# josl/kmerjs

Measured on AMD Instinct MI355X. Metric: k-mers/sec + distinct-kmers/sec, k=16 150bp synthetic FASTQ, 1/2/4/8 GPU, higher is better.
Workload: dtype u8; 1 GPU; C2: 10000000 synthetic 150bp reads per GPU, k=16, prefix 'ATGAC'; reads_per_gpu=10000000, mode=ordered (reference Map insertion order), k=16, prefix=ATGAC, bytes_per_gpu=3170000000, pipeline=off (steps in sequence), parallelism=dp1 (one GPU; no collective), backend=none

## Files before the change

### kmerjs_amd/csrc/kmer_api.hip

```cpp
#include "kmer_host.hpp"

using namespace kmerhip;

extern "C" {

const char *kmer_version(void) { return "kmerhip 0.2 (gfx950)"; }

const char *kmer_status_string(kmer_status s) {
    switch (s) {
    case KMER_OK: return "ok";
    case KMER_E_IO: return "i/o error";
    case KMER_E_BAD_PARAM: return "bad parameter";
    case KMER_E_OOM: return "out of memory";
    case KMER_E_DEVICE: return "device error";
    case KMER_E_TOO_MANY_KEYS: return "too many keys";
    case KMER_E_NONASCII: return "non-ASCII input";
    case KMER_E_LINE_TOO_LONG: return "line too long";
    case KMER_E_STATE: return "bad call sequence";
    }
    return "unknown";
}

const char *kmer_last_error(const kmer_ctx *ctx) { return ctx ? ctx->err.c_str() : "null context"; }

// ... 297 lines not shown
kmer_status kmer_feed_device(kmer_ctx *c, const void *d_bytes, size_t len, void *stream) {
    if (!c || (!d_bytes && len)) return KMER_E_BAD_PARAM;
    SETTLE(c);
    if (!c->open_stream) return fail(c, KMER_E_STATE, "feed without reset");
    if (hipSetDevice(c->device) != hipSuccess) return KMER_E_DEVICE;
    hipStream_t s = (hipStream_t)stream;
    if (s != c->stream) {
        HIPCHK(c, hipEventRecord(c->evw, s));
        HIPCHK(c, hipStreamWaitEvent(c->stream, c->evw, 0));
    }
    return feed(c, (const uint8_t *)d_bytes, len, c->stream);
}

kmer_status kmer_finish_device(kmer_ctx *c, kmer_result **out) {
    if (!c) return KMER_E_BAD_PARAM;
    SETTLE(c);
    if (hipSetDevice(c->device) != hipSuccess) return KMER_E_DEVICE;
    if (out) *out = nullptr;
    return finish(c, out);
}


kmer_status kmer_partial_device(kmer_ctx *c, const void **d_keys, const void **d_vals, uint64_t *n) {
    if (!c || !d_keys || !d_vals || !n) return KMER_E_BAD_PARAM;
    SETTLE(c);
    if (c->mode != MODE_PACKED && c->mode != MODE_WINDOWS)
        return fail(c, KMER_E_STATE, "configuration has no packed keys");
    if (c->wide) return fail(c, KMER_E_STATE, "keys of 64 bits or more (k - |P| >= 32) have no packed partials");
    if (hipSetDevice(c->device) != hipSuccess) return KMER_E_DEVICE;
    kmer_status st = apply_cross(c);
    if (st) return st;
// ... 1572 lines not shown
```

### kmerjs_amd/csrc/kmer_feed.hip

```cpp
#include "kmer_host.hpp"

namespace kmerhip {

kmer_status ensure_tiles(kmer_ctx *c, uint64_t n_tiles) {
    if (n_tiles <= c->tile_cap) return KMER_OK;
    const uint64_t cap = std::max<uint64_t>(n_tiles, 1024);
    hipStream_t s = c->stream;
    if (c->mode == MODE_TABLE) {
    } else if (c->mode == MODE_GENERAL || c->mode == MODE_WINDOWS) {
        HIPCHK(c, c->lb_cnt.ensure(cap, s));
        HIPCHK(c, c->lb_lnl.ensure(cap, s));
        HIPCHK(c, c->tp_cnt.ensure(cap, s));
        HIPCHK(c, c->tp_lnl.ensure(cap, s));
    } else {
        HIPCHK(c, c->tsum.ensure(cap, s));
        HIPCHK(c, c->tscan.ensure(cap, s));
        HIPCHK(c, c->bsum.ensure(cap / TSCAN_BLOCK + 2, s));
        HIPCHK(c, c->bscan.ensure(cap / TSCAN_BLOCK + 2, s));
        HIPCHK(c, c->hits.ensure(cap * HMAX, s));
        if (c->p.k > 32) HIPCHK(c, c->hits_hi.ensure(cap * HMAX, s));
    }
    c->tile_cap = cap;
    return KMER_OK;
}
// ... 47 lines not shown
    HIPCHK(c, hipStreamSynchronize(s));
    std::string key;
    for (uint64_t i = 0; i < n; ++i) {
        key.assign(keys.data() + i * k, recs[i].len);
        auto it = c->exotic.find(key);
        if (it == c->exotic.end()) {
            c->exotic.emplace(key, Ent{1, recs[i].order});
        } else {
            it->second.count += 1;
            it->second.first = std::min(it->second.first, recs[i].order);
        }
    }
    return KMER_OK;
}

kmer_status wait_tail(kmer_ctx *c, uint64_t seq, hipStream_t qs) {
    volatile uint64_t *flag = c->h_tail + 9;
    for (uint32_t i = 1;; ++i) {
        if (__atomic_load_n(flag, __ATOMIC_ACQUIRE) == seq) break;
        if ((i & 1023) == 0) {
            const hipError_t e = hipStreamQuery(qs);
            if (e == hipSuccess) {
                if (__atomic_load_n(flag, __ATOMIC_ACQUIRE) == seq) break;
                return fail(c, KMER_E_DEVICE, "chunk counters were not published");
            }
            if (e != hipErrorNotReady) HIPCHK(c, e);
        }
        __builtin_ia32_pause();
    }
    memcpy(c->h_small, (const void *)c->h_tail, 8 * 8);
    return KMER_OK;
}

static void take_chunk_stamps(kmer_ctx *c) {
    const uint64_t t0 = c->h_tail[TAIL_STAMP + STAMP_SCAN_START], t1 = c->h_tail[TAIL_STAMP + STAMP_SCAN_END],
                   t2 = c->h_tail[TAIL_STAMP + STAMP_FEED_END];
    c->scan_ms += (double)(int64_t)(t1 - t0) / c->clock_khz;
    c->feed_ms += (double)(int64_t)(t2 - t0) / c->clock_khz;
}

kmer_status flush_prep(kmer_ctx *c, hipStream_t s, uint32_t extra) {
    const uint32_t f = c->prep_flags | extra;
    if (!f) return KMER_OK;
    HIPCHK(c, launch_prep(c->d_pos, c->d_pos_saved, c->d_err, c->d_scal, f, c->prep_lines, c->d_stamp, s));
    c->prep_flags = 0;
// ... 50 lines not shown
    h.xbase = c->n_cross;
    h.xcap = c->xord.cap;
    uint64_t rcap = c->narrow ? c->rkey32.cap : c->rkey.cap;
    rcap = std::min<uint64_t>(rcap, c->rord.cap);
    if (c->wide) rcap = std::min<uint64_t>(rcap, c->rkeyh.cap);
    h.rcap = rcap;
}

kmer_status launch_chunk(kmer_ctx *c) {
    auto &p = c->pend;
    const hipStream_t s = p.s;
    uint64_t *stamp = c->d_stamp;
    if (c->planes) HIPCHK(c, launch_scan_planes(p.a, c->pargs, s));
    else HIPCHK(c, launch_scan_tiles(p.a, s));
    HIPCHK(c, launch_tile_reduce(c->tsum.p, p.n_tiles, c->bsum.p, stamp, s));
    if (p.n_blocks > TSCAN_INLINE_MAX) {
        TileSum zero;
        memset(&zero, 0, sizeof(zero));
        ROCPRIM_RUN(c, rocprim::exclusive_scan(t, b, c->bsum.p, c->bscan.p, zero, (size_t)p.n_blocks, TileSumOp(), s));
        HIPCHK(c, launch_tile_scan(c->tsum.p, p.n_tiles, c->bscan.p, true, p.init, c->tscan.p, s));
    } else {
        HIPCHK(c, launch_tile_scan(c->tsum.p, p.n_tiles, c->bsum.p, false, p.init, c->tscan.p, s));
    }
    p.h.seq = ++c->tail_seq;
    p.h.stamp = stamp;
    HIPCHK(c, launch_hits(p.h, s));
    if (c->mode == MODE_PACKED && !c->wide)
        HIPCHK(c, launch_cross_segsort_chunk(p.h.xord, p.h.xkey, p.h.xslot, p.h.xbase, p.h.xcap, c->d_xcount,
                                             c->d_cross_go, p.h.rkey, p.h.rkey32, p.h.rord, c->pbits, s));
    if (s != c->stream) {
        HIPCHK(c, hipEventRecord(c->evw, s));
        HIPCHK(c, hipStreamWaitEvent(c->stream, c->evw, 0));
    }
    return KMER_OK;
}

kmer_status scan_feed(kmer_ctx *c, const uint8_t *d, uint64_t len, uint32_t n_tiles, hipStream_t s) {
    const bool packed = c->mode == MODE_PACKED;
    kmer_status st;
// ... 729 lines not shown
```

### kmerjs_amd/csrc/kmer_finish.hip

```cpp
#include "kmer_host.hpp"

namespace kmerhip {

kmer_status apply_cross(kmer_ctx *c) {
    hipStream_t s = c->stream;
    const uint64_t n = c->n_cross;
    if (n == 0) return KMER_OK;
    uint32_t *k32 = c->narrow ? c->rkey32.p : nullptr;
    if (!c->long_seg) {
        HIPCHK(c, launch_cross_segsort(c->xord.p, c->xkey.p, c->xslot.p, n, c->rkey.p, k32, c->rord.p, c->pbits,
                                       c->fin_stamp, s));
        c->fin_stamp = nullptr;
    } else if (n <= XSMALL_MAX) {
        HIPCHK(c, launch_cross_sort_small(c->xslot.p, c->xord.p, c->xkey.p, n, c->rkey.p, k32, c->rord.p, s));
    } else {
        StreamPos pos;
        kmer_status st = read_pos(c, &pos);
        if (st) return st;
        HIPCHK(c, c->xord2.ensure(n, s));
        HIPCHK(c, c->xkey2.ensure(n, s));
        rocprim::double_buffer<uint64_t> ob(c->xord.p, c->xord2.p);
        rocprim::double_buffer<uint64_t> kb(c->xkey.p, c->xkey2.p);
        const int obits = std::min(64, bit_width(((pos.lines + 1) << (c->pbits + 1)) | ((2ull << c->pbits) - 1ull)));
        ROCPRIM_RUN(c, rocprim::radix_sort_pairs(t, b, ob, kb, (size_t)n, 0, obits, s));
// ... 38 lines not shown
    rocprim::counting_iterator<uint32_t> iota(0u);
    ROCPRIM_RUN(c, rocprim::radix_sort_pairs(t, b, c->rkey.p, c->rkey2.p, iota, c->ridx2.p, (size_t)n, 0, 64, s));
    HIPCHK(c, launch_gather_u64(c->rkeyh.p, c->ridx2.p, n, c->whA.p, s));
    const int hbits = (int)c->kbits - 64 + 1;
    ROCPRIM_RUN(c, rocprim::radix_sort_pairs(t, b, c->whA.p, c->whB.p, c->ridx2.p, c->ridx3.p, (size_t)n, 0, hbits, s));
    HIPCHK(c, launch_gather_u64(c->rkey.p, c->ridx3.p, n, c->rkey2.p, s));
    HIPCHK(c, hipMemsetD32Async((hipDeviceptr_t)c->hcnt.p, 1, n, s));
    HIPCHK(c, launch_heads_wide(c->whB.p, c->rkey2.p, c->ridx3.p, n, 1ull << (c->kbits - 64), c->hcnt.p, s));
    return KMER_OK;
}

bool bucket_route(const kmer_ctx *c, bool with_counts) {
    return c->narrow && c->kbits <= BKT_LOW + 11 && !with_counts && !(c->p.flags & KMER_FLAG_SORT_FINISH);
}

kmer_status bucket_heads(kmer_ctx *c, uint64_t n, bool partial) {
    hipStream_t s = c->stream;
    const uint32_t shift = std::min<uint32_t>(c->kbits, BKT_LOW);
    const uint32_t nb = 1u << (c->kbits - shift);
    const uint64_t nblk64 = (n + BKT_EPB_HOST - 1) / BKT_EPB_HOST;
    if (nblk64 > 0x7FFFFFFFull) return fail(c, KMER_E_BAD_PARAM, "too many hits");
    const uint32_t nblk = (uint32_t)nblk64;
    const uint32_t invalid = 1u << c->kbits;
    uint64_t *stamp = c->fin_stamp;
    c->fin_stamp = nullptr;
    const uint64_t cap = bucket_cap(n, nb);
    if (!c->bkt_counted && (uint64_t)nb * cap <= 0x7FFFFFFFull) {
        HIPCHK(c, c->pkey16.ensure((uint64_t)nb * cap, s));
        HIPCHK(c, c->ridx2.ensure((uint64_t)nb * cap, s));
        if (!c->bcur.p) {
            HIPCHK(c, c->bcur.ensure((uint64_t)BKT_MAX * BKT_CUR_STRIDE, s));
            HIPCHK(c, hipMemsetAsync(c->bcur.p, 0, (uint64_t)BKT_MAX * BKT_CUR_STRIDE * sizeof(uint32_t), s));
        }
        HIPCHK(c, launch_bucket_onepass(c->rkey32.p, n, invalid, shift, nb, nblk, (uint32_t)cap, c->bcur.p, c->pkey16.p,
                                        c->ridx2.p, c->hcnt.p, c->d_err, stamp, s));
        HIPCHK(c, launch_bucket_heads(c->pkey16.p, c->ridx2.p, nullptr, nb, shift, c->hcnt.p, c->bcur.p, (uint32_t)cap, n,
                                      c->d_err, s));
        c->bkt_check = true;
        c->bkt_n = n;
        c->bkt_partial = partial;
        return KMER_OK;
    }
// ... 102 lines not shown
        HIPCHK(c, c->cnt_out.ensure(n, s));
        HIPCHK(c, c->first.ensure(n, s));
    }
    const uint64_t invalid = c->kbits >= 63 ? ~0ull : (1ull << c->kbits);
    kmer_status st;
    const bool bucket = bucket_route(c, with_counts);
    if (c->wide)
        st = sort_and_heads_wide(c, n);
    else if (bucket)
        st = bucket_heads(c, n, partial);
    else if (c->narrow)
        st = sort_and_heads<uint32_t>(c, c->rkey32.p, c->rkey32b.p, n, with_counts);
    else
        st = sort_and_heads<uint64_t>(c, c->rkey.p, c->rkey2.p, n, with_counts);
    if (st) return st;
    const uint64_t nbe = emit_blocks(n);
    HIPCHK(c, c->ecnt.ensure(nbe, s));
    HIPCHK(c, launch_head_count(c->hcnt.p, n, c->ecnt.p, s));
    EmitArgs e;
    memset(&e, 0, sizeof(e));
    e.ecnt = c->ecnt.p;
    if (nbe > EMIT_DIRECT_MAX) {
        HIPCHK(c, c->epre.ensure(nbe, s));
        ROCPRIM_RUN(c, rocprim::exclusive_scan(t, b, c->ecnt.p, c->epre.p, (uint64_t)0, (size_t)nbe,
                                               rocprim::plus<uint64_t>(), s));
        e.epre = c->epre.p;
    }
    e.hcnt = c->hcnt.p;
    e.hrec = with_counts ? c->hrec.p : nullptr;
    e.rkey32 = c->narrow ? c->rkey32.p : nullptr;
    e.rkey64 = c->narrow ? nullptr : c->rkey.p;
    e.rkeyh = c->wide ? c->rkeyh.p : nullptr;
    e.rord = c->rord.p;
    e.n = n;
    e.invalid_key = invalid;
    e.nuniq = c->d_nuniq;
    e.nuniq_host = c->d_tail + TAIL_NUNIQ;
    e.host_out = c->d_tail;
    e.err = c->d_err;
    e.stamp = c->fin_emit;
    e.k = c->p.k;
    e.plen = (uint32_t)c->prefix.size();
    e.partial = partial ? 1u : 0u;
    memcpy(e.P, c->prefix.data(), std::min<size_t>(c->prefix.size(), sizeof(e.P)));
    e.keys_out = c->keys_out.p;
    e.cnt_out = c->cnt_out.p;
    e.first_out = c->first.p;
    e.ukey = c->ukey.p;
    e.uval = c->uval.p;
    HIPCHK(c, launch_emit(e, s));
    if (!sync) {
        c->out_pending = true;
        return KMER_OK;
    }
    HIPCHK(c, hipStreamSynchronize(s));
    *nu_out = c->h_tail[TAIL_NUNIQ];
    bool redo = false;
    st = bucket_observe(c, &redo);
// ... 213 lines not shown
}

kmer_status read_pos(kmer_ctx *c, StreamPos *pos) {
    kmer_status st = settle(c);
    if (st) return st;
    st = flush_prep(c, c->stream, 0);
    if (st) return st;
    HIPCHK(c, hipMemcpyAsync(c->h_small + 8, c->d_pos, sizeof(StreamPos), hipMemcpyDeviceToHost, c->stream));
    HIPCHK(c, hipStreamSynchronize(c->stream));
    memcpy(pos, c->h_small + 8, sizeof(StreamPos));
    return KMER_OK;
}

kmer_status finish(kmer_ctx *c, kmer_result **out) {
    if (!c->open_stream) return fail(c, KMER_E_STATE, "finish without reset/feed");
    kmer_status st = settle(c);
    if (st) return st;
    const bool stamped = c->mode == MODE_PACKED && c->n_hits > 0 && bucket_route(c, false) && !(c->n_cross && c->long_seg);
    const bool events = !stamped;
    c->fin_stamp = c->fin_emit = stamped ? c->d_stamp : nullptr;
    if (events) HIPCHK(c, hipEventRecord(c->ev2, c->stream));
    uint64_t nu = 0;
    c->n_out = 0;
    const bool sync = out || c->p.max_keys;
    if (c->mode == MODE_PACKED || c->mode == MODE_WINDOWS) {
        st = apply_cross(c);
        if (st) return st;
        if (c->mode == MODE_WINDOWS && !c->prefix.empty() && c->win_slots) {
            st = compact_windows(c);
            if (st) return st;
        }
// ... 33 lines not shown
```

### kmerjs_amd/csrc/kmer_host.hpp

```cpp
#pragma once
#include <hip/hip_runtime.h>
#include <rocprim/device/device_radix_sort.hpp>
#include <rocprim/device/device_scan.hpp>
#include <rocprim/device/device_select.hpp>
#include <rocprim/iterator/counting_iterator.hpp>
#include <rocprim/iterator/transform_iterator.hpp>

#include <algorithm>
#include <condition_variable>
#include <cstdio>
#include <deque>
#include <mutex>
#include <functional>
#include <cstdlib>
#include <cstring>
#include <memory>
#include <string>
#include <thread>
#include <unordered_map>
#include <vector>

#include "../../include/kmer_api.h"
#include "kmer_internal.hpp"

// ... 228 lines not shown
    uint64_t gm_n = 0;
    DBuf<uint8_t> gm_keys, gm_keys2;
    DBuf<uint64_t> gm_cnt, gm_cnt2, gm_first, gm_first2, gm_h1, gm_h2, gm_h1b, gm_h2b;
    DBuf<uint32_t> gm_idx, gm_idx2, gm_head, gm_gid, gm_start;
    DBuf<unsigned int> gm_flag;
    DBuf<uint64_t> gkeys, gkeys2;
    DBuf<Agg> gvals, gvals2;
    double t_ms[7] = {};
    hipEvent_t fa_ev[2] = {nullptr, nullptr};
    int n_cu = 0;
    uint64_t *d_stamp = nullptr;
    double clock_khz = 0.0;
    uint64_t *fin_stamp = nullptr;
    uint64_t *fin_emit = nullptr;
    bool finish_stamped = false;
    hipEvent_t ev0 = nullptr, ev1 = nullptr, ev2 = nullptr, ev3 = nullptr;
    hipEvent_t evw = nullptr;
    double scan_ms = 0.0, feed_ms = 0.0, finish_ms = 0.0;
    bool fasta = false;
    DBuf<FaTile> fa_t, fa_x;
    DBuf<uint8_t> fa_out[2];
    uint32_t fa_flip = 0;
    uint64_t fa_lines = 0;
    bool progress_any = false;
    uint64_t progress_hw = 0;
};

namespace kmerhip {


// ... 73 lines not shown
    virtual void progress(uint64_t *done, uint64_t *total) = 0;
    virtual bool next(const uint8_t **p, uint64_t *n, kmer_status *st, std::string *err) = 0;
    virtual void release(const uint8_t *) {}
};

kmer_status ensure_tiles(kmer_ctx *c, uint64_t n_tiles);
kmer_status upload(kmer_ctx *c, void *dst, const void *src, size_t n, hipStream_t s);
kmer_status general_append(kmer_ctx *c, const uint8_t *d, uint64_t nrec, hipStream_t s);
kmer_status general_merge(kmer_ctx *c);
kmer_status general_finish(kmer_ctx *c);
kmer_status general_to_host(kmer_ctx *c);
kmer_status ensure_ovf(kmer_ctx *c, uint64_t n, hipStream_t s);
kmer_status ensure_records(kmer_ctx *c, uint64_t n);
kmer_status drain_records(kmer_ctx *c, const uint8_t *d_data, uint64_t n, hipStream_t s);
kmer_status wait_tail(kmer_ctx *c, uint64_t seq, hipStream_t qs);
bool bucket_route(const kmer_ctx *c, bool with_counts);
kmer_status flush_prep(kmer_ctx *c, hipStream_t s, uint32_t extra);
kmer_status check_err(kmer_ctx *c, uint32_t e);
kmer_status ensure_rank_arrays(kmer_ctx *c, uint64_t need, uint64_t keep, hipStream_t s);
kmer_status ensure_cross(kmer_ctx *c, uint64_t need, hipStream_t s);
void bind_hits(kmer_ctx *c, HitArgs &h);
kmer_status launch_chunk(kmer_ctx *c);
kmer_status scan_feed(kmer_ctx *c, const uint8_t *d, uint64_t len, uint32_t n_tiles, hipStream_t s);
kmer_status settle(kmer_ctx *c);
kmer_status two_pass_prefix(kmer_ctx *c, const uint8_t *d, uint64_t len, uint32_t n_tiles, hipStream_t s);
kmer_status collect_lines(kmer_ctx *c, const uint8_t *d, uint64_t len, uint32_t n_tiles, hipStream_t s,
                          uint64_t *nlines_out);
kmer_status general_feed(kmer_ctx *c, const uint8_t *d, uint64_t len, uint32_t n_tiles, hipStream_t s);
kmer_status chunk_lines(kmer_ctx *c, const uint8_t *d, uint64_t len, uint32_t n_tiles, hipStream_t s, bool check_len,
                        uint64_t *n_nl_out, uint64_t *n_seq_out);
// ... 36 lines not shown
```

### kmerjs_amd/csrc/kmer_internal.hpp

```cpp
#pragma once
#include <hip/hip_runtime.h>
#include <stdint.h>

namespace kmerhip {


constexpr int TPB = 256;
constexpr int BPT = 64;
constexpr int TILE = TPB * BPT;
constexpr int FH = 64;
constexpr int BH = 80;
constexpr int KMAX_PACKED = 32;
constexpr int KMAX_TILE = 64;
constexpr int KMAX_DENSE = 32;
constexpr uint32_t MAXREL = (1u << 23) - 1;
constexpr uint32_t PBITS_DEFAULT = 23, PBITS_LONG = 40;
constexpr uint32_t NL_SLOTS = 1024;

enum : uint32_t {
    ERR_NONASCII = 1u << 0,
    ERR_LINE_TOO_LONG = 1u << 1,
    ERR_LOOKBACK_TIMEOUT = 1u << 2,
    ERR_REC_OVERFLOW = 1u << 3,
    ERR_LINE_OVERFLOW = 1u << 4,
// ... 132 lines not shown
    uint64_t rec_cap;
    unsigned int *err;
    const uint8_t *data;
    uint64_t len;
    uint64_t *scal;
    unsigned int *ticket;
    unsigned long long *chunk_hits, *chunk_cross, *ends_open;
    unsigned int *cross_go;
    uint64_t *host_out;
    uint64_t seq;
    uint64_t *stamp;
};

enum : uint32_t { STAMP_SCAN_START = 0, STAMP_SCAN_END = 1, STAMP_FEED_END = 2, STAMP_FINISH_START = 3, STAMP_WORDS = 4 };
enum : uint32_t { TAIL_NUNIQ = 8, TAIL_SEQ = 9, TAIL_ERR = 10, TAIL_STAMP = 11, TAIL_FIN_START = 14, TAIL_FIN_END = 15,
                  TAIL_WORDS = 16 };
__device__ __forceinline__ void stamp_now(uint64_t *stamp, uint32_t which) {
    if (stamp && blockIdx.x == 0 && threadIdx.x == 0) stamp[which] = wall_clock64();
}

struct HeadRec {
    uint64_t key;
    uint64_t count;
};

struct EmitArgs {
    const uint32_t *hcnt;
    const HeadRec *hrec;
    const uint32_t *rkey32;
    const uint64_t *rkey64;
    const uint64_t *rkeyh;
// ... 125 lines not shown
    uint64_t *rord;
    const uint8_t *P, *RP;
    Record *recs;
    unsigned long long *rec_count;
    uint64_t rec_cap;
    unsigned int *err;
};
hipError_t launch_dense_windows(const DenseArgs &a, bool write, hipStream_t s);

hipError_t launch_lines(const TileArgs &a, bool lookback, hipStream_t s);
hipError_t launch_scan_tiles(const ScanArgs &a, hipStream_t s);
hipError_t launch_scan_planes(const ScanArgs &a, const PlaneArgs &pa, hipStream_t s);
hipError_t launch_hits(const HitArgs &a, hipStream_t s);
hipError_t launch_tile_reduce(const TileSum *in, uint32_t n, TileSum *bsum, uint64_t *stamp, hipStream_t s);
hipError_t launch_tile_scan(const TileSum *in, uint32_t n, const TileSum *bsum, bool bsum_scanned, TileSum init,
                            TileSum *out, hipStream_t s);
enum : uint32_t { PREP_RESET = 1, PREP_SETPOS = 2, PREP_SAVE = 4, PREP_ZERO = 8 };
hipError_t launch_prep(StreamPos *pos, StreamPos *saved, unsigned int *err, uint64_t *scal, uint32_t flags,
                       uint64_t lines, uint64_t *stamp, hipStream_t s);
hipError_t launch_tile_aggregate(const uint8_t *data, uint64_t len, uint32_t n_tiles, uint64_t *agg_cnt,
                                 uint64_t *agg_lnl, unsigned int *err, hipStream_t s);
hipError_t launch_windows(const WindowArgs &a, uint32_t grid, hipStream_t s);
hipError_t launch_cross_scatter(const uint32_t *slot, const uint64_t *ord, const uint64_t *key, uint64_t n,
                                uint64_t *rkey, uint32_t *rkey32, uint64_t *rord, hipStream_t s);
hipError_t launch_cross_sort_small(const uint32_t *slot, const uint64_t *ord, const uint64_t *key, uint64_t n,
                                   uint64_t *rkey, uint32_t *rkey32, uint64_t *rord, hipStream_t s);
constexpr uint64_t XSMALL_MAX = 16384;
hipError_t launch_cross_segsort(uint64_t *ord, uint64_t *key, const uint32_t *slot, uint64_t n, uint64_t *rkey,
                                uint32_t *rkey32, uint64_t *rord, uint32_t pbits, uint64_t *stamp, hipStream_t s);
hipError_t launch_cross_segsort_chunk(uint64_t *ord, uint64_t *key, const uint32_t *slot, uint64_t xbase, uint64_t xcap,
                                      const unsigned long long *count, const unsigned int *go, uint64_t *rkey,
                                      uint32_t *rkey32, uint64_t *rord, uint32_t pbits, hipStream_t s);
hipError_t launch_heads(const uint64_t *skey, const uint32_t *srank, uint64_t n, uint64_t invalid_key,
                        const uint64_t *rcnt, HeadRec *hrec, uint32_t *hcnt, hipStream_t s);
hipError_t launch_heads_sparse(const uint64_t *skey64, const uint32_t *skey32, const uint32_t *srank, uint64_t n,
                               uint64_t invalid_key, uint32_t *hcnt, hipStream_t s);
hipError_t launch_heads32(const uint32_t *skey, const uint32_t *srank, uint64_t n, uint32_t invalid_key,
                          const uint64_t *rcnt, HeadRec *hrec, uint32_t *hcnt, hipStream_t s);
hipError_t launch_emit(const EmitArgs &a, hipStream_t s);
hipError_t launch_head_count(const uint32_t *hcnt, uint64_t n, uint32_t *ecnt, hipStream_t s);
uint64_t emit_blocks(uint64_t n);
constexpr uint64_t EMIT_DIRECT_MAX = 4096;
hipError_t launch_gather_u64(const uint64_t *src, const uint32_t *idx, uint64_t n, uint64_t *dst, hipStream_t s);
constexpr uint64_t CP_BLOCK = 4096;
hipError_t launch_compact_count(const uint32_t *k32, const uint64_t *k64, uint64_t n, uint64_t invalid, uint32_t *bcnt,
                                hipStream_t s);
hipError_t launch_compact_write(const uint32_t *k32, const uint64_t *k64, const uint64_t *ord, uint64_t n,
                                uint64_t invalid, const uint64_t *boff, uint32_t *o32, uint64_t *o64, uint64_t *oord,
                                hipStream_t s);
hipError_t launch_cross_wide_fix(const uint32_t *xslot, uint64_t n, const uint64_t *xkeyl, const uint64_t *xkeyh,
                                 uint64_t *rkey, uint64_t *rkeyh, hipStream_t s);
hipError_t launch_heads_wide(const uint64_t *shi, const uint64_t *slo, const uint32_t *srank, uint64_t n,
                             uint64_t invalid_hi, uint32_t *hcnt, hipStream_t s);
constexpr uint32_t BKT_LOW = 14;
constexpr uint32_t BKT_MAX = 2048;
constexpr uint32_t BKT_EPB_HOST = 4096;
// ... 592 lines not shown
```

### kmerjs_amd/csrc/kmer_kernels.hip

```cpp
#include "kmer_device.hpp"

#include <algorithm>
#include <cstring>

namespace kmerhip {

__device__ __forceinline__ uint32_t align4(uint32_t hi, uint32_t lo, uint32_t sel) {
    return __builtin_amdgcn_alignbyte(hi, lo, sel);
}

__device__ __forceinline__ void set_info(unsigned int *err, unsigned int bit) {
    if (!(__hip_atomic_load(err, __ATOMIC_RELAXED, __HIP_MEMORY_SCOPE_AGENT) & bit)) atomicOr(err, bit);
}

__device__ __forceinline__ uint32_t not_nl_bits(uint32_t x) {
    return ((x ^ 0x0A0A0A0Au) + 0x7F7F7F7Fu) & 0x80808080u;
}

__device__ __forceinline__ uint32_t not_nl_bits_xad(uint32_t x, uint32_t k0a, uint32_t k7f) {
    uint32_t r;
    asm("v_xad_u32 %0, %1, %2, %3" : "=v"(r) : "v"(x), "v"(k0a), "s"(k7f));
    return r & 0x80808080u;
}

// ... 1075 lines not shown
                                                          uint64_t *stamp) {
    stamp_now(stamp, STAMP_SCAN_END);
    const uint32_t base = blockIdx.x * TSCAN_BLOCK;
    TileSum v = ts_zero();
#pragma unroll
    for (uint32_t i = 0; i < TSCAN_BLOCK / 256; ++i) {
        const uint32_t t = base + i * 256 + threadIdx.x;
        if (t < n) v = tile_sum_op(v, in[t]);
    }
    TileSum tot;
    (void)ts_block_scan(v, &tot);
    if (threadIdx.x == 0) bsum[blockIdx.x] = tot;
}

__global__ __launch_bounds__(256) void tile_scan_kernel(const TileSum *in, uint32_t n, const TileSum *bsum,
                                                        uint32_t bsum_scanned, TileSum init, TileSum *out) {
    const uint32_t b = blockIdx.x;
    TileSum pre;
    if (bsum_scanned) {
        pre = tile_sum_op(init, bsum[b]);
    } else {
        TileSum v = ts_zero();
        for (uint32_t j = threadIdx.x; j < b; j += 256) v = tile_sum_op(v, bsum[j]);
        TileSum tot;
        (void)ts_block_scan(v, &tot);
        pre = tile_sum_op(init, tot);
    }
    const uint32_t t0 = b * TSCAN_BLOCK + threadIdx.x * 4;
    TileSum x[4];
    TileSum acc = ts_zero();
#pragma unroll
    for (int i = 0; i < 4; ++i) {
        x[i] = t0 + i < n ? in[t0 + i] : ts_zero();
        acc = tile_sum_op(acc, x[i]);
    }
    TileSum tot;
    TileSum ex = tile_sum_op(pre, ts_block_scan(acc, &tot));
#pragma unroll
    for (int i = 0; i < 4; ++i) {
        if (t0 + i < n) out[t0 + i] = ex;
        ex = tile_sum_op(ex, x[i]);
    }
}

__global__ void prep_kernel(StreamPos *pos, StreamPos *saved, unsigned int *err, uint64_t *scal, uint32_t flags,
                            uint64_t lines, uint64_t *stamp) {
    if (threadIdx.x != 0 || blockIdx.x != 0) return;
    StreamPos p = *pos;
    if (flags & PREP_RESET) {
        p.lines = p.unused = p.ends_open = p.pad = 0;
        *err = 0;
    }
    if (flags & PREP_SETPOS) {
        p.lines = lines;
        p.unused = p.ends_open = p.pad = 0;
    }
// ... 1203 lines not shown
    __shared__ uint32_t skey[BKT_EPB];
    __shared__ uint32_t srank[BKT_EPB];
    __shared__ uint32_t wtot[4];
    for (uint32_t b = threadIdx.x; b < nb; b += 256) cnt[b] = 0;
    __syncthreads();
    const uint64_t base = (uint64_t)blockIdx.x * BKT_EPB;
    for (uint32_t j = 4 * threadIdx.x; j < BKT_EPB; j += 4 * 256) {
        const uint64_t i = base + j;
        if (i + 4 <= n) *(uint4 *)(hcnt + i) = make_uint4(0, 0, 0, 0);
        else for (uint64_t t = i; t < n; ++t) hcnt[t] = 0;
    }
    uint32_t kk[BKT_EPB / 256], li[BKT_EPB / 256];
#pragma unroll
    for (uint32_t u = 0; u < BKT_EPB / 256; ++u) {
        const uint64_t i = base + u * 256 + threadIdx.x;
        kk[u] = i < n ? key[i] : invalid;
        li[u] = kk[u] != invalid ? atomicAdd(&cnt[kk[u] >> shift], 1u) : 0u;
    }
    __syncthreads();
    uint32_t loc[BKT_MAX / 256], sum = 0;
#pragma unroll
    for (uint32_t u = 0; u < BKT_MAX / 256; ++u) {
        const uint32_t b = threadIdx.x * (BKT_MAX / 256) + u;
        loc[u] = b < nb ? cnt[b] : 0u;
        sum += loc[u];
    }
    uint32_t gpos[BKT_MAX / 256];
#pragma unroll
    for (uint32_t u = 0; u < BKT_MAX / 256; ++u) {
        const uint32_t b = threadIdx.x * (BKT_MAX / 256) + u;
        gpos[u] = b < nb && loc[u] ? atomicAdd(cur + (uint64_t)b * BKT_CUR_STRIDE, loc[u]) : 0u;
// ... 84 lines not shown
            }
        }
    }
    __syncthreads();
    for (uint32_t j = threadIdx.x; j < nk; j += blockDim.x) {
        const uint32_t c = cnt[j];
        if (c) {
            const uint32_t r = minr[j];
            if (r < n) hcnt[r] = c;
            else atomicOr(err, ERR_BKT_RANK);
        }
    }
}

constexpr uint32_t EMIT_RPB = 1024;
__global__ __launch_bounds__(256) void head_count_kernel(const uint32_t *hcnt, uint64_t n, uint32_t *ecnt) {
    __shared__ uint32_t ws[4];
    const uint64_t r0 = (uint64_t)blockIdx.x * EMIT_RPB + 4 * threadIdx.x;
    uint32_t c = 0;
    if (r0 + 4 <= n) {
        const uint4 v = *(const uint4 *)(hcnt + r0);
        c = (v.x != 0) + (v.y != 0) + (v.z != 0) + (v.w != 0);
    } else {
        for (uint64_t r = r0; r < n; ++r) c += hcnt[r] != 0;
    }
    c = wave_incl_sum(c);
    if ((threadIdx.x & 63) == 63) ws[threadIdx.x >> 6] = c;
    __syncthreads();
    if (threadIdx.x == 0) ecnt[blockIdx.x] = ws[0] + ws[1] + ws[2] + ws[3];
}

__global__ __launch_bounds__(256) void emit_kernel(EmitArgs a) {
    __shared__ __attribute__((aligned(16))) uint8_t kbuf[256 * KMAX_TILE];
    __shared__ uint32_t s_w[EMIT_RPB / 256][4];
    __shared__ uint64_t s_pre;
    __shared__ uint32_t s_wp[4];
    const uint64_t n = a.n;
    const uint32_t k = a.k, plen = a.plen;
    const bool staged = !a.partial && (k & 3);
    const int tid = threadIdx.x, lane = tid & 63, wid = tid >> 6;
    const uint64_t rb = (uint64_t)blockIdx.x * EMIT_RPB;
    constexpr int NR = EMIT_RPB / 256;
    uint32_t hcr[NR];
    unsigned long long hm[NR];
#pragma unroll
    for (int i = 0; i < NR; ++i) {
        const uint64_t r = rb + 256 * i + tid;
        hcr[i] = r < n ? a.hcnt[r] : 0u;
        hm[i] = __ballot(hcr[i] != 0);
        if (lane == 0) s_w[i][wid] = (uint32_t)__popcll(hm[i]);
    }
    uint64_t ekey[NR], ecnt[NR], efirst[NR], ekeyh[NR];
#pragma unroll
    for (int i = 0; i < NR; ++i) {
        const uint64_t r = rb + 256 * i + tid;
        ekey[i] = ecnt[i] = efirst[i] = ekeyh[i] = 0;
        if (hcr[i]) {
            if (a.hrec) {
                const HeadRec v = a.hrec[r];
                ekey[i] = v.key;
                ecnt[i] = v.count;
            } else {
                ekey[i] = a.rkey32 ? (uint64_t)a.rkey32[r] : a.rkey64[r];
                if (a.rkeyh) ekeyh[i] = a.rkeyh[r];
                ecnt[i] = hcr[i];
            }
            efirst[i] = a.rord[r];
        }
    }
    if (a.epre) {
        if (tid == 0) s_pre = a.epre[blockIdx.x];
    } else {
        uint32_t p = 0;
        for (uint32_t j = tid; j < blockIdx.x; j += 256) p += a.ecnt[j];
        p = wave_incl_sum(p);
        if (lane == 63) s_wp[wid] = p;
    }
    __syncthreads();
    if (!a.epre && tid == 0) s_pre = (uint64_t)s_wp[0] + s_wp[1] + s_wp[2] + s_wp[3];
// ... 16 lines not shown
        const uint64_t oend = o0 + rt;
        if (r == n - 1) {
            *a.nuniq = o64 + f;
            if (a.host_out) {
                a.host_out[TAIL_ERR] = __hip_atomic_load(a.err, __ATOMIC_RELAXED, __HIP_MEMORY_SCOPE_AGENT);
                if (a.stamp) a.host_out[TAIL_FIN_START] = a.stamp[STAMP_FINISH_START];
            }
            if (a.nuniq_host) {
                *a.nuniq_host = o64 + f;
                __threadfence_system();
            }
        }
        const uint64_t o = o64;
        if (f) {
            const uint64_t key = ekey[i], cnt = ecnt[i], keyh = ekeyh[i], first = efirst[i];
            if (a.partial) {
                a.ukey[o] = key;
                Agg v;
                v.first = first;
                v.count = cnt;
                a.uval[o] = v;
            } else {
                a.cnt_out[o] = cnt;
                a.first_out[o] = first;
                uint8_t *out = staged ? kbuf + (o - o0) * k : a.keys_out + o * k;
                const uint32_t nw = (k + 3) / 4;
                uint32_t w0 = 0, w1 = 0, w2 = 0;
                for (int w = 0; w < KMAX_TILE / 4; ++w) {
                    if ((uint32_t)w >= nw) break;
                    uint32_t v = 0;
#pragma unroll
// ... 2 lines not shown
                        uint32_t ch = 0;
                        if (pos < plen) {
                            ch = a.P[pos];
                        } else if (pos < k) {
                            const uint32_t sh = 2 * (k - 1 - pos);
                            const uint32_t b = (uint32_t)(sh < 64 ? key >> sh : keyh >> (sh - 64)) & 3u;
                            ch = (0x54474341u >> (8 * b)) & 0xFFu;
                        }
                        v |= ch << (8 * j);
                    }
                    if (k == 16) {
                        if (w == 0) w0 = v;
                        else if (w == 1) w1 = v;
                        else if (w == 2) w2 = v;
                        else *(uint4 *)out = make_uint4(w0, w1, w2, v);
                    } else if ((k & 3) == 0) {
                        *(uint32_t *)(out + 4 * w) = v;
                    } else {
                        for (uint32_t b = 4 * w; b < k && b < 4 * (uint32_t)w + 4; ++b)
                            out[b] = (uint8_t)(v >> (8 * (b & 3)));
                    }
                }
            }
        }
        if (staged) {
            __syncthreads();
            const uint64_t g0 = (uint64_t)o0 * k, g1 = (uint64_t)oend * k;
            const uint64_t a0 = (g0 + 3) & ~3ull, a1 = g1 & ~3ull;
            if (a0 >= a1) {
                for (uint64_t g = g0 + threadIdx.x; g < g1; g += 256) a.keys_out[g] = kbuf[g - g0];
            } else {
// ... 269 lines not shown

hipError_t launch_hits(const HitArgs &a, hipStream_t s) {
    const dim3 grid((a.n_tiles + 4 * HTPW - 1) / (4 * HTPW));
    if (a.wide) hipLaunchKernelGGL(hit_kernel<true>, grid, dim3(256), 0, s, a);
    else hipLaunchKernelGGL(hit_kernel<false>, grid, dim3(256), 0, s, a);
    hipLaunchKernelGGL(hit_overflow_kernel, dim3(64), dim3(256), 0, s, a);
    return hipGetLastError();
}

hipError_t launch_tile_reduce(const TileSum *in, uint32_t n, TileSum *bsum, uint64_t *stamp, hipStream_t s) {
    hipLaunchKernelGGL(tile_reduce_kernel, dim3((n + TSCAN_BLOCK - 1) / TSCAN_BLOCK), dim3(256), 0, s, in, n, bsum,
                       stamp);
    return hipGetLastError();
}
hipError_t launch_tile_scan(const TileSum *in, uint32_t n, const TileSum *bsum, bool bsum_scanned, TileSum init,
                            TileSum *out, hipStream_t s) {
    hipLaunchKernelGGL(tile_scan_kernel, dim3((n + TSCAN_BLOCK - 1) / TSCAN_BLOCK), dim3(256), 0, s, in, n, bsum,
                       bsum_scanned ? 1u : 0u, init, out);
    return hipGetLastError();
}
hipError_t launch_prep(StreamPos *pos, StreamPos *saved, unsigned int *err, uint64_t *scal, uint32_t flags,
                       uint64_t lines, uint64_t *stamp, hipStream_t s) {
    hipLaunchKernelGGL(prep_kernel, dim3(1), dim3(64), 0, s, pos, saved, err, scal, flags, lines, stamp);
    return hipGetLastError();
}
hipError_t launch_tile_aggregate(const uint8_t *data, uint64_t len, uint32_t n_tiles, uint64_t *agg_cnt,
                                 uint64_t *agg_lnl, unsigned int *err, hipStream_t s) {
    hipLaunchKernelGGL(tile_aggregate_kernel, dim3(n_tiles), dim3(TPB), 0, s, data, len, agg_cnt, agg_lnl, err);
    return hipGetLastError();
}

hipError_t launch_windows(const WindowArgs &a, uint32_t grid, hipStream_t s) {
    hipLaunchKernelGGL(windows_kernel, dim3(grid), dim3(256), 0, s, a);
// ... 230 lines not shown
hipError_t launch_bucket_onepass(const uint32_t *key, uint64_t n, uint32_t invalid, uint32_t shift, uint32_t nb,
                                 uint32_t nblk, uint32_t cap, uint32_t *cur, uint16_t *pkey, uint32_t *prank,
                                 uint32_t *hcnt, unsigned int *err, uint64_t *stamp, hipStream_t s) {
    if (nb == 0 || nb > BKT_MAX || (uint64_t)nb * cap > 0x7FFFFFFFull) return hipErrorInvalidValue;
    hipLaunchKernelGGL(bucket_onepass_kernel, dim3(nblk), dim3(256), 0, s, key, n, invalid, shift, nb, cap, cur, pkey,
                       prank, hcnt, err, stamp);
    return hipGetLastError();
}
hipError_t launch_bucket_heads(const uint16_t *pkey, const uint32_t *prank, const uint32_t *bbase, uint32_t nb,
                               uint32_t shift, uint32_t *hcnt, uint32_t *cur, uint32_t cap, uint64_t n,
                               unsigned int *err, hipStream_t s) {
    hipLaunchKernelGGL(bucket_heads_kernel, dim3(nb), dim3(1024), 0, s, pkey, prank, bbase, shift, hcnt, cur, cap, n,
                       err);
    return hipGetLastError();
}
uint64_t emit_blocks(uint64_t n) { return (n + EMIT_RPB - 1) / EMIT_RPB; }
hipError_t launch_head_count(const uint32_t *hcnt, uint64_t n, uint32_t *ecnt, hipStream_t s) {
    if (n) hipLaunchKernelGGL(head_count_kernel, dim3((uint32_t)emit_blocks(n)), dim3(256), 0, s, hcnt, n, ecnt);
    return hipGetLastError();
}
hipError_t launch_emit(const EmitArgs &a, hipStream_t s) {
    if (a.n) hipLaunchKernelGGL(emit_kernel, dim3((uint32_t)emit_blocks(a.n)), dim3(256), 0, s, a);
    return hipGetLastError();
}
hipError_t launch_merge_prep(const uint64_t *keys, const Agg *vals, uint64_t n, uint64_t *rkey, uint32_t *rkey32,
                             uint64_t *rord, uint64_t *rcnt, uint32_t *ridx, hipStream_t s) {
    if (n)
        hipLaunchKernelGGL(merge_prep_kernel, dim3(grid_for(n)), dim3(256), 0, s, keys, vals, n, rkey, rkey32, rord, rcnt,
                           ridx);
    return hipGetLastError();
}
hipError_t launch_xpart_hist(const uint64_t *rkey, const uint32_t *rkey32, uint64_t n, uint64_t invalid,
                             uint32_t kbits, uint32_t world, uint32_t nblk, uint32_t *H, hipStream_t s) {
    if (world == 0 || world > XP_MAXW || nblk == 0) return hipErrorInvalidValue;
    hipLaunchKernelGGL(xpart_hist_kernel, dim3(nblk), dim3(256), 0, s, rkey, rkey32, n, invalid, kbits, world, nblk, H);
    return hipGetLastError();
}
// ... 74 lines not shown
```

Baseline: 3793 billion k-mers/s.

## Start finish early from tile-scan totals and add lean emit kernel variant

The tile-scan kernel now publishes the hit, cross and overflow totals to a host-visible tail word. When conditions allow, finish waits only on this early word and queues rank_finish before settling, so the finish work overlaps the hits kernel instead of waiting for the whole chunk; on a mismatch it falls back to the normal path. A templated lean emit/head-count variant handles the narrow, 4-aligned-k case with more rows per block and no staging buffer. Host polling also throttles hipStreamQuery to a time interval. The speculative path adds extra state and validation logic.

After: 3813 billion k-mers/s, median of 6. No clear change (+0.5%).

```diff
diff --git a/kmerjs_amd/csrc/kmer_api.hip b/kmerjs_amd/csrc/kmer_api.hip
--- a/kmerjs_amd/csrc/kmer_api.hip
+++ b/kmerjs_amd/csrc/kmer_api.hip
@@ -335,7 +335,7 @@
 
 kmer_status kmer_finish_device(kmer_ctx *c, kmer_result **out) {
     if (!c) return KMER_E_BAD_PARAM;
-    SETTLE(c);
+    if (!c->group.empty()) return fail(c, KMER_E_STATE, "single-device call on a group context");
     if (hipSetDevice(c->device) != hipSuccess) return KMER_E_DEVICE;
     if (out) *out = nullptr;
     return finish(c, out);
diff --git a/kmerjs_amd/csrc/kmer_feed.hip b/kmerjs_amd/csrc/kmer_feed.hip
--- a/kmerjs_amd/csrc/kmer_feed.hip
+++ b/kmerjs_amd/csrc/kmer_feed.hip
@@ -1,4 +1,6 @@
 #include "kmer_host.hpp"
+
+#include <chrono>
 
 namespace kmerhip {
 
@@ -85,11 +87,18 @@
     return KMER_OK;
 }
 
-kmer_status wait_tail(kmer_ctx *c, uint64_t seq, hipStream_t qs) {
-    volatile uint64_t *flag = c->h_tail + 9;
+constexpr int WAIT_QUERY_MS = 2;
+static kmer_status wait_word(kmer_ctx *c, uint32_t word, uint64_t seq, hipStream_t qs) {
+    using clk = std::chrono::steady_clock;
+    volatile uint64_t *flag = c->h_tail + word;
+    clk::time_point next{};
     for (uint32_t i = 1;; ++i) {
         if (__atomic_load_n(flag, __ATOMIC_ACQUIRE) == seq) break;
         if ((i & 1023) == 0) {
+            const clk::time_point now = clk::now();
+            if (next == clk::time_point{}) next = now + std::chrono::milliseconds(WAIT_QUERY_MS);
+            if (now < next) continue;
+            next = now + std::chrono::milliseconds(WAIT_QUERY_MS);
             const hipError_t e = hipStreamQuery(qs);
             if (e == hipSuccess) {
                 if (__atomic_load_n(flag, __ATOMIC_ACQUIRE) == seq) break;
@@ -99,7 +108,20 @@
         }
         __builtin_ia32_pause();
     }
+    return KMER_OK;
+}
+kmer_status wait_tail(kmer_ctx *c, uint64_t seq, hipStream_t qs) {
+    const kmer_status st = wait_word(c, TAIL_SEQ, seq, qs);
+    if (st) return st;
     memcpy(c->h_small, (const void *)c->h_tail, 8 * 8);
+    return KMER_OK;
+}
+kmer_status wait_early(kmer_ctx *c, uint64_t *hits, uint64_t *cross, uint64_t *ovf) {
+    const kmer_status st = wait_word(c, TAIL_EARLY_SEQ, c->pend.h.seq, c->pend.s);
+    if (st) return st;
+    *hits = c->h_tail[TAIL_EARLY_HITS];
+    *cross = c->h_tail[TAIL_EARLY_CROSS];
+    *ovf = c->h_tail[TAIL_EARLY_OVF];
     return KMER_OK;
 }
 
@@ -180,15 +202,17 @@
     if (c->planes) HIPCHK(c, launch_scan_planes(p.a, c->pargs, s));
     else HIPCHK(c, launch_scan_tiles(p.a, s));
     HIPCHK(c, launch_tile_reduce(c->tsum.p, p.n_tiles, c->bsum.p, stamp, s));
+    p.h.seq = ++c->tail_seq;
     if (p.n_blocks > TSCAN_INLINE_MAX) {
         TileSum zero;
         memset(&zero, 0, sizeof(zero));
         ROCPRIM_RUN(c, rocprim::exclusive_scan(t, b, c->bsum.p, c->bscan.p, zero, (size_t)p.n_blocks, TileSumOp(), s));
-        HIPCHK(c, launch_tile_scan(c->tsum.p, p.n_tiles, c->bscan.p, true, p.init, c->tscan.p, s));
+        HIPCHK(c, launch_tile_scan(c->tsum.p, p.n_tiles, c->bscan.p, true, p.init, c->tscan.p, c->d_ovf_count, c->d_tail,
+                                   p.h.seq, s));
     } else {
-        HIPCHK(c, launch_tile_scan(c->tsum.p, p.n_tiles, c->bsum.p, false, p.init, c->tscan.p, s));
-    }
-    p.h.seq = ++c->tail_seq;
+        HIPCHK(c, launch_tile_scan(c->tsum.p, p.n_tiles, c->bsum.p, false, p.init, c->tscan.p, c->d_ovf_count, c->d_tail,
+                                   p.h.seq, s));
+    }
     p.h.stamp = stamp;
     HIPCHK(c, launch_hits(p.h, s));
     if (c->mode == MODE_PACKED && !c->wide)
diff --git a/kmerjs_amd/csrc/kmer_finish.hip b/kmerjs_amd/csrc/kmer_finish.hip
--- a/kmerjs_amd/csrc/kmer_finish.hip
+++ b/kmerjs_amd/csrc/kmer_finish.hip
@@ -76,6 +76,11 @@
     return c->narrow && c->kbits <= BKT_LOW + 11 && !with_counts && !(c->p.flags & KMER_FLAG_SORT_FINISH);
 }
 
+static bool bucket_onepass_route(const kmer_ctx *c, uint64_t n) {
+    const uint32_t nb = 1u << (c->kbits - std::min<uint32_t>(c->kbits, BKT_LOW));
+    return !c->bkt_counted && (uint64_t)nb * bucket_cap(n, nb) <= 0x7FFFFFFFull;
+}
+
 kmer_status bucket_heads(kmer_ctx *c, uint64_t n, bool partial) {
     hipStream_t s = c->stream;
     const uint32_t shift = std::min<uint32_t>(c->kbits, BKT_LOW);
@@ -87,7 +92,7 @@
     uint64_t *stamp = c->fin_stamp;
     c->fin_stamp = nullptr;
     const uint64_t cap = bucket_cap(n, nb);
-    if (!c->bkt_counted && (uint64_t)nb * cap <= 0x7FFFFFFFull) {
+    if (bucket_onepass_route(c, n)) {
         HIPCHK(c, c->pkey16.ensure((uint64_t)nb * cap, s));
         HIPCHK(c, c->ridx2.ensure((uint64_t)nb * cap, s));
         if (!c->bcur.p) {
@@ -220,11 +225,17 @@
     else
         st = sort_and_heads<uint64_t>(c, c->rkey.p, c->rkey2.p, n, with_counts);
     if (st) return st;
-    const uint64_t nbe = emit_blocks(n);
-    HIPCHK(c, c->ecnt.ensure(nbe, s));
-    HIPCHK(c, launch_head_count(c->hcnt.p, n, c->ecnt.p, s));
     EmitArgs e;
     memset(&e, 0, sizeof(e));
+    e.hrec = with_counts ? c->hrec.p : nullptr;
+    e.rkey32 = c->narrow ? c->rkey32.p : nullptr;
+    e.rkeyh = c->wide ? c->rkeyh.p : nullptr;
+    e.k = c->p.k;
+    e.partial = partial ? 1u : 0u;
+    const bool lean = emit_lean(e);
+    const uint64_t nbe = emit_blocks(n, lean);
+    HIPCHK(c, c->ecnt.ensure(nbe, s));
+    HIPCHK(c, launch_head_count(c->hcnt.p, n, lean, c->ecnt.p, s));
     e.ecnt = c->ecnt.p;
     if (nbe > EMIT_DIRECT_MAX) {
         HIPCHK(c, c->epre.ensure(nbe, s));
@@ -233,10 +244,7 @@
         e.epre = c->epre.p;
     }
     e.hcnt = c->hcnt.p;
-    e.hrec = with_counts ? c->hrec.p : nullptr;
-    e.rkey32 = c->narrow ? c->rkey32.p : nullptr;
     e.rkey64 = c->narrow ? nullptr : c->rkey.p;
-    e.rkeyh = c->wide ? c->rkeyh.p : nullptr;
     e.rord = c->rord.p;
     e.n = n;
     e.invalid_key = invalid;
@@ -245,9 +253,7 @@
     e.host_out = c->d_tail;
     e.err = c->d_err;
     e.stamp = c->fin_emit;
-    e.k = c->p.k;
     e.plen = (uint32_t)c->prefix.size();
-    e.partial = partial ? 1u : 0u;
     memcpy(e.P, c->prefix.data(), std::min<size_t>(c->prefix.size(), sizeof(e.P)));
     e.keys_out = c->keys_out.p;
     e.cnt_out = c->cnt_out.p;
@@ -491,7 +497,38 @@
 
 kmer_status finish(kmer_ctx *c, kmer_result **out) {
     if (!c->open_stream) return fail(c, KMER_E_STATE, "finish without reset/feed");
-    kmer_status st = settle(c);
+    kmer_status st;
+    bool queued = false;
+    uint64_t n_early = 0;
+    const uint64_t seq0 = c->tail_seq;
+    if (c->pend.active && !c->early_finish_off && !out && !c->p.max_keys && c->mode == MODE_PACKED && !c->wide && !c->long_seg &&
+        c->n_cross == 0 && bucket_route(c, false)) {
+        uint64_t hits = 0, cross = 0, ovf = 0;
+        const HitArgs &h = c->pend.h;
+        if (wait_early(c, &hits, &cross, &ovf) == KMER_OK && hits > 0 && ovf <= h.ovf_cap && h.xbase + cross <= h.xcap &&
+            c->n_hits + hits <= h.rcap && bucket_onepass_route(c, c->n_hits + hits)) {
+            n_early = c->n_hits + hits;
+            uint64_t nu0 = 0;
+            c->fin_stamp = c->fin_emit = c->d_stamp;
+            st = rank_finish(c, n_early, false, false, &nu0, false);
+            c->fin_stamp = c->fin_emit = nullptr;
+            if (st) return st;
+            queued = true;
+        }
+    }
+    st = settle(c);
+    if (queued) {
+        if (!st && c->tail_seq == seq0 && c->n_hits == n_early && c->n_cross == 0 && !c->long_seg) {
+            c->n_out = 0;
+            c->timing_pending = true;
+            c->finish_stamped = true;
+            c->open_stream = false;
+            return KMER_OK;
+        }
+        c->out_pending = false;
+        c->bkt_check = false;
+        if (c->long_seg) c->early_finish_off = true;
+    }
     if (st) return st;
     const bool stamped = c->mode == MODE_PACKED && c->n_hits > 0 && bucket_route(c, false) && !(c->n_cross && c->long_seg);
     const bool events = !stamped;
diff --git a/kmerjs_amd/csrc/kmer_host.hpp b/kmerjs_amd/csrc/kmer_host.hpp
--- a/kmerjs_amd/csrc/kmer_host.hpp
+++ b/kmerjs_amd/csrc/kmer_host.hpp
@@ -266,6 +266,7 @@
     uint64_t *fin_stamp = nullptr;
     uint64_t *fin_emit = nullptr;
     bool finish_stamped = false;
+    bool early_finish_off = false;
     hipEvent_t ev0 = nullptr, ev1 = nullptr, ev2 = nullptr, ev3 = nullptr;
     hipEvent_t evw = nullptr;
     double scan_ms = 0.0, feed_ms = 0.0, finish_ms = 0.0;
@@ -369,6 +370,7 @@
 kmer_status ensure_records(kmer_ctx *c, uint64_t n);
 kmer_status drain_records(kmer_ctx *c, const uint8_t *d_data, uint64_t n, hipStream_t s);
 kmer_status wait_tail(kmer_ctx *c, uint64_t seq, hipStream_t qs);
+kmer_status wait_early(kmer_ctx *c, uint64_t *hits, uint64_t *cross, uint64_t *ovf);
 bool bucket_route(const kmer_ctx *c, bool with_counts);
 kmer_status flush_prep(kmer_ctx *c, hipStream_t s, uint32_t extra);
 kmer_status check_err(kmer_ctx *c, uint32_t e);
diff --git a/kmerjs_amd/csrc/kmer_internal.hpp b/kmerjs_amd/csrc/kmer_internal.hpp
--- a/kmerjs_amd/csrc/kmer_internal.hpp
+++ b/kmerjs_amd/csrc/kmer_internal.hpp
@@ -170,7 +170,8 @@
 
 enum : uint32_t { STAMP_SCAN_START = 0, STAMP_SCAN_END = 1, STAMP_FEED_END = 2, STAMP_FINISH_START = 3, STAMP_WORDS = 4 };
 enum : uint32_t { TAIL_NUNIQ = 8, TAIL_SEQ = 9, TAIL_ERR = 10, TAIL_STAMP = 11, TAIL_FIN_START = 14, TAIL_FIN_END = 15,
-                  TAIL_WORDS = 16 };
+                  TAIL_EARLY_HITS = 16, TAIL_EARLY_CROSS = 17, TAIL_EARLY_OVF = 18, TAIL_EARLY_SEQ = 19,
+                  TAIL_WORDS = 20 };
 __device__ __forceinline__ void stamp_now(uint64_t *stamp, uint32_t which) {
     if (stamp && blockIdx.x == 0 && threadIdx.x == 0) stamp[which] = wall_clock64();
 }
@@ -326,7 +327,8 @@
 hipError_t launch_hits(const HitArgs &a, hipStream_t s);
 hipError_t launch_tile_reduce(const TileSum *in, uint32_t n, TileSum *bsum, uint64_t *stamp, hipStream_t s);
 hipError_t launch_tile_scan(const TileSum *in, uint32_t n, const TileSum *bsum, bool bsum_scanned, TileSum init,
-                            TileSum *out, hipStream_t s);
+                            TileSum *out, const unsigned long long *ovf_count, uint64_t *early, uint64_t seq,
+                            hipStream_t s);
 enum : uint32_t { PREP_RESET = 1, PREP_SETPOS = 2, PREP_SAVE = 4, PREP_ZERO = 8 };
 hipError_t launch_prep(StreamPos *pos, StreamPos *saved, unsigned int *err, uint64_t *scal, uint32_t flags,
                        uint64_t lines, uint64_t *stamp, hipStream_t s);
@@ -350,8 +352,9 @@
 hipError_t launch_heads32(const uint32_t *skey, const uint32_t *srank, uint64_t n, uint32_t invalid_key,
                           const uint64_t *rcnt, HeadRec *hrec, uint32_t *hcnt, hipStream_t s);
 hipError_t launch_emit(const EmitArgs &a, hipStream_t s);
-hipError_t launch_head_count(const uint32_t *hcnt, uint64_t n, uint32_t *ecnt, hipStream_t s);
-uint64_t emit_blocks(uint64_t n);
+hipError_t launch_head_count(const uint32_t *hcnt, uint64_t n, bool lean, uint32_t *ecnt, hipStream_t s);
+bool emit_lean(const EmitArgs &a);
+uint64_t emit_blocks(uint64_t n, bool lean);
 constexpr uint64_t EMIT_DIRECT_MAX = 4096;
 hipError_t launch_gather_u64(const uint64_t *src, const uint32_t *idx, uint64_t n, uint64_t *dst, hipStream_t s);
 constexpr uint64_t CP_BLOCK = 4096;
diff --git a/kmerjs_amd/csrc/kmer_kernels.hip b/kmerjs_amd/csrc/kmer_kernels.hip
--- a/kmerjs_amd/csrc/kmer_kernels.hip
+++ b/kmerjs_amd/csrc/kmer_kernels.hip
@@ -1113,7 +1113,9 @@
 }
 
 __global__ __launch_bounds__(256) void tile_scan_kernel(const TileSum *in, uint32_t n, const TileSum *bsum,
-                                                        uint32_t bsum_scanned, TileSum init, TileSum *out) {
+                                                        uint32_t bsum_scanned, TileSum init, TileSum *out,
+                                                        const unsigned long long *ovf_count, uint64_t *early,
+                                                        uint64_t seq) {
     const uint32_t b = blockIdx.x;
     TileSum pre;
     if (bsum_scanned) {
@@ -1139,6 +1141,13 @@
     for (int i = 0; i < 4; ++i) {
         if (t0 + i < n) out[t0 + i] = ex;
         ex = tile_sum_op(ex, x[i]);
+        if (early && t0 + i == n - 1) {
+            early[TAIL_EARLY_HITS] = ex.nh;
+            early[TAIL_EARLY_CROSS] = ex.nx;
+            early[TAIL_EARLY_OVF] = *ovf_count;
+            __threadfence_system();
+            __hip_atomic_store(early + TAIL_EARLY_SEQ, seq, __ATOMIC_RELEASE, __HIP_MEMORY_SCOPE_SYSTEM);
+        }
     }
 }
 
@@ -2372,7 +2381,7 @@
 #pragma unroll
     for (uint32_t u = 0; u < BKT_EPB / 256; ++u) {
         const uint64_t i = base + u * 256 + threadIdx.x;
-        kk[u] = i < n ? key[i] : invalid;
+        kk[u] = i < n ? min(key[i], invalid) : invalid;
         li[u] = kk[u] != invalid ? atomicAdd(&cnt[kk[u] >> shift], 1u) : 0u;
     }
     __syncthreads();
@@ -2487,15 +2496,21 @@
 }
 
 constexpr uint32_t EMIT_RPB = 1024;
+constexpr uint32_t EMIT_RPB_LEAN = 1536;
+template <uint32_t RPB>
 __global__ __launch_bounds__(256) void head_count_kernel(const uint32_t *hcnt, uint64_t n, uint32_t *ecnt) {
     __shared__ uint32_t ws[4];
-    const uint64_t r0 = (uint64_t)blockIdx.x * EMIT_RPB + 4 * threadIdx.x;
     uint32_t c = 0;
-    if (r0 + 4 <= n) {
-        const uint4 v = *(const uint4 *)(hcnt + r0);
-        c = (v.x != 0) + (v.y != 0) + (v.z != 0) + (v.w != 0);
-    } else {
-        for (uint64_t r = r0; r < n; ++r) c += hcnt[r] != 0;
+#pragma unroll
+    for (uint32_t off = 0; off < RPB; off += 1024) {
+        if (off + 4 * threadIdx.x >= RPB) break;
+        const uint64_t r0 = (uint64_t)blockIdx.x * RPB + off + 4 * threadIdx.x;
+        if (r0 + 4 <= n) {
+            const uint4 v = *(const uint4 *)(hcnt + r0);
+            c += (v.x != 0) + (v.y != 0) + (v.z != 0) + (v.w != 0);
+        } else {
+            for (uint64_t r = r0; r < n; ++r) c += hcnt[r] != 0;
+        }
     }
     c = wave_incl_sum(c);
     if ((threadIdx.x & 63) == 63) ws[threadIdx.x >> 6] = c;
@@ -2503,17 +2518,21 @@
     if (threadIdx.x == 0) ecnt[blockIdx.x] = ws[0] + ws[1] + ws[2] + ws[3];
 }
 
+template <uint32_t RPB, bool LEAN>
 __global__ __launch_bounds__(256) void emit_kernel(EmitArgs a) {
-    __shared__ __attribute__((aligned(16))) uint8_t kbuf[256 * KMAX_TILE];
-    __shared__ uint32_t s_w[EMIT_RPB / 256][4];
+    __shared__ __attribute__((aligned(16))) uint8_t kbuf[LEAN ? 16 : 256 * KMAX_TILE];
+    __shared__ uint32_t s_w[RPB / 256][4];
     __shared__ uint64_t s_pre;
     __shared__ uint32_t s_wp[4];
     const uint64_t n = a.n;
     const uint32_t k = a.k, plen = a.plen;
-    const bool staged = !a.partial && (k & 3);
+    const bool partial = !LEAN && a.partial;
+    const bool staged = !LEAN && !partial && (k & 3);
+    const HeadRec *const hrec = LEAN ? nullptr : a.hrec;
+    const uint64_t *const rkeyh = LEAN ? nullptr : a.rkeyh;
     const int tid = threadIdx.x, lane = tid & 63, wid = tid >> 6;
-    const uint64_t rb = (uint64_t)blockIdx.x * EMIT_RPB;
-    constexpr int NR = EMIT_RPB / 256;
+    const uint64_t rb = (uint64_t)blockIdx.x * RPB;
+    constexpr int NR = RPB / 256;
     uint32_t hcr[NR];
     unsigned long long hm[NR];
 #pragma unroll
@@ -2529,13 +2548,13 @@
         const uint64_t r = rb + 256 * i + tid;
         ekey[i] = ecnt[i] = efirst[i] = ekeyh[i] = 0;
         if (hcr[i]) {
-            if (a.hrec) {
-                const HeadRec v = a.hrec[r];
+            if (hrec) {
+                const HeadRec v = hrec[r];
                 ekey[i] = v.key;
                 ecnt[i] = v.count;
             } else {
-                ekey[i] = a.rkey32 ? (uint64_t)a.rkey32[r] : a.rkey64[r];
-                if (a.rkeyh) ekeyh[i] = a.rkeyh[r];
+                ekey[i] = (LEAN || a.rkey32) ? (uint64_t)a.rkey32[r] : a.rkey64[r];
+                if (rkeyh) ekeyh[i] = rkeyh[r];
                 ecnt[i] = hcr[i];
             }
             efirst[i] = a.rord[r];
@@ -2582,7 +2601,7 @@
         const uint64_t o = o64;
         if (f) {
             const uint64_t key = ekey[i], cnt = ecnt[i], keyh = ekeyh[i], first = efirst[i];
-            if (a.partial) {
+            if (partial) {
                 a.ukey[o] = key;
                 Agg v;
                 v.first = first;
@@ -2615,7 +2634,7 @@
                         else if (w == 1) w1 = v;
                         else if (w == 2) w2 = v;
                         else *(uint4 *)out = make_uint4(w0, w1, w2, v);
-                    } else if ((k & 3) == 0) {
+                    } else if (LEAN || (k & 3) == 0) {
                         *(uint32_t *)(out + 4 * w) = v;
                     } else {
                         for (uint32_t b = 4 * w; b < k && b < 4 * (uint32_t)w + 4; ++b)
@@ -2915,9 +2934,10 @@
     return hipGetLastError();
 }
 hipError_t launch_tile_scan(const TileSum *in, uint32_t n, const TileSum *bsum, bool bsum_scanned, TileSum init,
-                            TileSum *out, hipStream_t s) {
+                            TileSum *out, const unsigned long long *ovf_count, uint64_t *early, uint64_t seq,
+                            hipStream_t s) {
     hipLaunchKernelGGL(tile_scan_kernel, dim3((n + TSCAN_BLOCK - 1) / TSCAN_BLOCK), dim3(256), 0, s, in, n, bsum,
-                       bsum_scanned ? 1u : 0u, init, out);
+                       bsum_scanned ? 1u : 0u, init, out, ovf_count, early, seq);
     return hipGetLastError();
 }
 hipError_t launch_prep(StreamPos *pos, StreamPos *saved, unsigned int *err, uint64_t *scal, uint32_t flags,
@@ -3178,13 +3198,24 @@
                        err);
     return hipGetLastError();
 }
-uint64_t emit_blocks(uint64_t n) { return (n + EMIT_RPB - 1) / EMIT_RPB; }
-hipError_t launch_head_count(const uint32_t *hcnt, uint64_t n, uint32_t *ecnt, hipStream_t s) {
-    if (n) hipLaunchKernelGGL(head_count_kernel, dim3((uint32_t)emit_blocks(n)), dim3(256), 0, s, hcnt, n, ecnt);
+bool emit_lean(const EmitArgs &a) {
+    return a.rkey32 && !a.hrec && !a.rkeyh && !a.partial && (a.k & 3) == 0;
+}
+uint64_t emit_blocks(uint64_t n, bool lean) {
+    const uint64_t rpb = lean ? EMIT_RPB_LEAN : EMIT_RPB;
+    return (n + rpb - 1) / rpb;
+}
+hipError_t launch_head_count(const uint32_t *hcnt, uint64_t n, bool lean, uint32_t *ecnt, hipStream_t s) {
+    const dim3 g((uint32_t)emit_blocks(n, lean));
+    if (n && lean) hipLaunchKernelGGL(head_count_kernel<EMIT_RPB_LEAN>, g, dim3(256), 0, s, hcnt, n, ecnt);
+    else if (n) hipLaunchKernelGGL(head_count_kernel<EMIT_RPB>, g, dim3(256), 0, s, hcnt, n, ecnt);
     return hipGetLastError();
 }
 hipError_t launch_emit(const EmitArgs &a, hipStream_t s) {
-    if (a.n) hipLaunchKernelGGL(emit_kernel, dim3((uint32_t)emit_blocks(a.n)), dim3(256), 0, s, a);
+    const bool lean = emit_lean(a);
+    const dim3 g((uint32_t)emit_blocks(a.n, lean));
+    if (a.n && lean) hipLaunchKernelGGL((emit_kernel<EMIT_RPB_LEAN, true>), g, dim3(256), 0, s, a);
+    else if (a.n) hipLaunchKernelGGL((emit_kernel<EMIT_RPB, false>), g, dim3(256), 0, s, a);
     return hipGetLastError();
 }
 hipError_t launch_merge_prep(const uint64_t *keys, const Agg *vals, uint64_t n, uint64_t *rkey, uint32_t *rkey32,
```
